# oneam/h264bsd

Hardware: AMD Instinct MI355X
Metric: 1080p macroblocks/s (higher is better)
Workload: dtype u8; 1 GPU; 256 concurrent copies of test_1920x1080.h264 per GPU (73 pictures x 8160 MB), kernel-only replay from HBM-resident frame jobs, inter+intra reconstruction + in-loop deblocking; streams_per_gpu=256, parallelism=streams/1, stream_groups=1, row_bands=library default (engine.hip TailConfig)

## Files before the change

### h264bsd_amd/csrc/engine.hip

```cpp
#include <hip/hip_runtime.h>
#include <stdio.h>
#include <stdlib.h>
#include <string.h>
#include <deque>
#include <memory>
#include <mutex>
#include <vector>
#include <algorithm>
#include "kernels.hip.h"
#include "kernels/k_tensor_out.hip.h"
#include "kernels/k_tensor_aa.hip.h"
#include "kernels/k_tensor_roi.hip.h"
#include "kernels/k_tensor_remap.hip.h"
#include "kernels/k_motion.hip.h"
#include "kernels/region_common.hip.h"
#include "kernels/k_region_stats.hip.h"
#include "kernels/k_keep.hip.h"
#include "kernels/k_blend.hip.h"
#include "kernels/k_region_change.hip.h"
#include "kernels/k_region_shift.hip.h"
#include "kernels/k_cell_maps.hip.h"
#include "kernels/k_cell_boxes.hip.h"
#include "engine.h"
#include "hip_owned.h"
// ... 293 lines not shown
    d.dbki = reinterpret_cast<const uint16_t *>(dev_blob + h->dbk_off);
    d.n_dbk = h->n_dbk;
    d.dbk = dev_dbk;
    d.cur = dev_frames + (size_t)h->cur_slot * frame_bytes;
    d.n_mbs = h->n_mbs;
    d.n_levels = h->n_intra_levels;
    d.wmb = h->width_mbs;
    d.wmb_magic = (uint32_t)(0x100000000ull / (h->width_mbs ? h->width_mbs : 1u)) + 1u;
    d.hmb = h->height_mbs;
    d.any_deblock = h->any_deblock;
    {
        const TailConfig tc = tail_config();
        const bool heavy = h->n_intra * 4u > h->n_mbs;
        d.heavy = heavy ? 1 : 0;
        d.dbk_bands = bands_for(h->height_mbs, heavy ? tc.dbk_rows_heavy : tc.dbk_rows_light);
        d.intra_bands = h->intra_down_deps ? 1 : bands_for(h->height_mbs, heavy ? tc.intra_rows_heavy : tc.intra_rows_light);
    }
    d.err = dev_err;
    d.conv_src = nullptr; d.conv_dst = nullptr; d.conv_fmt = 0; d.conv_pad = 0;
    for (uint32_t k = 0; k < FJ_MAX_SLOTS; k++) d.slot[k] = k < h->n_slots ? dev_frames + (size_t)k * frame_bytes : nullptr;
    if (shape) {
        shape->n_frames++;
        shape->max_mbs = std::max(shape->max_mbs, h->n_mbs);
        shape->max_copy = std::max(shape->max_copy, h->n_copy);
        shape->max_gen = std::max(shape->max_gen, h->n_gen);
        shape->max_gen_uni = std::max(shape->max_gen_uni, h->n_gen_uniform);
        shape->max_gen_quad = std::max(shape->max_gen_quad, h->n_gen_quad);
        shape->max_gen_rest = std::max(shape->max_gen_rest, h->n_gen - h->n_gen_uniform - h->n_gen_quad);
        shape->max_dbk = std::max(shape->max_dbk, h->n_dbk);
        shape->any_deblock |= h->any_deblock != 0;
        shape->max_levels = std::max(shape->max_levels, h->n_intra_levels);
        shape->max_w = std::max<uint32_t>(shape->max_w, h->width_mbs);
        shape->max_h = std::max<uint32_t>(shape->max_h, h->height_mbs);
        shape->any_tail |= h->n_intra_levels != 0 || h->any_deblock != 0;
        shape->n_heavy += d.heavy;
        if (h->any_deblock) (d.heavy ? shape->want_heavy : shape->want_light)[0] = std::max<uint32_t>((d.heavy ? shape->want_heavy : shape->want_light)[0], d.dbk_bands);
        if (h->n_intra_levels) (d.heavy ? shape->want_heavy : shape->want_light)[1] = std::max<uint32_t>((d.heavy ? shape->want_heavy : shape->want_light)[1], d.intra_bands);
        if (h->n_intra_levels && h->intra_down_deps) shape->intra_whole = true;
    }
}

struct TickTimers { Event ev[6]; Event sev[5]; bool on = false; bool copy_timed = false; unsigned mask = 31u; };

static void launch_kdbk(hipStream_t st, const FrameDesc *d_desc, const TickShape &s, uint32_t launches[5])
{
    hipLaunchKernelGGL(h264k::k_dbk, dim3((s.max_dbk + 64 * DBK_WG_WAVES - 1) / (64 * DBK_WG_WAVES), s.n_frames), dim3(64 * DBK_WG_WAVES), 0, st, d_desc);
    if (launches) launches[2]++;
}
template <int PATH> static void launch_inter(hipStream_t st, const FrameDesc *d_desc, uint32_t n_max, uint32_t n_frames)
{
#if INTER_LANE_BLOCKS
    if constexpr (PATH == 0) {
        if (n_max) hipLaunchKernelGGL(h264k::k_recon_inter_lb, dim3((n_max + INTER_LB_CHUNK - 1) / INTER_LB_CHUNK, n_frames), dim3(64), 0, st, d_desc);
    } else
#endif
    {
    constexpr uint32_t per_wg = INTER_WG_WAVES * h264k::inter_per_wave<PATH>();
    if (n_max) hipLaunchKernelGGL(h264k::k_recon_inter<PATH>, dim3((n_max + per_wg - 1) / per_wg, n_frames), dim3(64 * INTER_WG_WAVES), 0, st, d_desc);
    }
}
std::mutex g_tail_lds_mu;
size_t g_tail_lds[2][2][MAX_DEVICES] = {};
static int tail_prepare(hipStream_t st, int which, const BandPlan &bp, const void *fn, uint32_t **tickets)
{
    const bool banded = bp.bands > 1;
    *tickets = banded ? tickets_for(st) : nullptr;
    if (banded && !*tickets) return -1;
    int dev = 0;
    HIP_TRY(hipGetDevice(&dev));
    std::lock_guard<std::mutex> lk(g_tail_lds_mu);
    if (bp.lds > g_tail_lds[which][banded][dev]) {
        HIP_TRY(hipFuncSetAttribute(fn, hipFuncAttributeMaxDynamicSharedMemorySize, (int)bp.lds));
        g_tail_lds[which][banded][dev] = bp.lds;
    }
    return 0;
}

int launch_tick(hipStream_t st, const FrameDesc *d_desc, const TickShape &s, TickTimers *tt, uint32_t launches[5],
                unsigned stages = 7u, const SideLane *side = nullptr, unsigned long long *prof = nullptr)
{
    const bool timed = tt && tt->on;
    const unsigned tmask = timed ? tt->mask : 0u;
    auto boundary = [&](unsigned i) -> int {
        if ((((tmask << 1) | tmask) >> i) & 1u) HIP_TRY(hipEventRecord(tt->ev[i], st));
        return 0;
    };
    if (boundary(0)) return -1;
    const bool do_dbk = (stages & 4u) && s.any_deblock && s.max_dbk;
    const bool do_copy = (stages & 1u) && s.max_copy;
    const bool aside = side && side->stream && do_dbk;
    const bool copy_aside = aside && do_copy && side->copy_stream;
    if (tt) tt->copy_timed = false;
    auto launch_copy = [&](hipStream_t cs) {
        hipLaunchKernelGGL(h264k::k_copy, dim3(std::min<uint32_t>((s.max_copy + 3) / 4, COPY_WGS), s.n_frames), dim3(256), 0, cs, d_desc);
        if (launches) launches[0]++;
    };
    if (aside) {
        HIP_TRY(hipEventRecord(side->fork, st));
        HIP_TRY(hipStreamWaitEvent(side->stream, side->fork, 0));
        if (copy_aside) {
            const bool ctimed = timed && (tmask & 1u) && tt->sev[3] && tt->sev[4];
            if (tt) tt->copy_timed = ctimed;
            HIP_TRY(hipStreamWaitEvent(side->copy_stream, side->fork, 0));
            if (ctimed) HIP_TRY(hipEventRecord(tt->sev[3], side->copy_stream));
            launch_copy(side->copy_stream);
            if (ctimed) HIP_TRY(hipEventRecord(tt->sev[4], side->copy_stream));
// ... 1402 lines not shown
```

### h264bsd_amd/csrc/kernels/inter_lane_block.hip.h

```cpp
#pragma once
namespace h264k {

constexpr uint32_t lb_sel(int c) { return 0x0C000C00u | (uint32_t)c | ((uint32_t)(c + 1) << 16); }
#define LB_CP(row, c) as_s2((c) <= 6 ? perm((row)[1], (row)[0], lb_sel((c) <= 6 ? (c) : 0)) : perm((row)[2], (row)[1], lb_sel((c) <= 6 ? 0 : (c) - 4)))
#define LB_RND5(x) pk_clip(pk(0), pk(255), ((x) + pk(16)) >> pk(5))
__device__ __forceinline__ s2 lb_tap6(s2 a, s2 b, s2 c, s2 d, s2 e, s2 f) { return a + f - pk(5) * (b + e) + pk(20) * (c + d); }
__device__ __forceinline__ int lb_dot2(s2 a, s2 b, int c)
{
#if defined(__HIP_DEVICE_COMPILE__)
    return __builtin_amdgcn_sdot2(a, b, c, false);
#else
    return (int)a.x * b.x + (int)a.y * b.y + c;
#endif
}
__device__ __forceinline__ s2 lb_avg(s2 a, s2 b) { return (a + b + pk(1)) >> pk(1); }
__device__ __forceinline__ s2 lb_pick(bool c, s2 a, s2 b) { return as_s2(c ? as_u32(a) : as_u32(b)); }
__device__ __forceinline__ void lb_hsum(const uint32_t row[3], s2 &h01, s2 &h23)
{
    const s2 c0 = LB_CP(row, 0), c1 = LB_CP(row, 1), c2 = LB_CP(row, 2), c3 = LB_CP(row, 3), c4 = LB_CP(row, 4), c5 = LB_CP(row, 5), c6 = LB_CP(row, 6), c7 = LB_CP(row, 7);
    h01 = lb_tap6(c0, c1, c2, c3, c4, c5); h23 = lb_tap6(c2, c3, c4, c5, c6, c7);
}

__device__ __forceinline__ void lb_luma_whole(const uint32_t rw[9][3], s2 o[4][2])
{
// ... 108 lines not shown
}
__device__ __forceinline__ void lb_residual_pk(const uint32_t y[8], const uint32_t c[8], int qp_y, int qp_c, int dc, uint32_t r[4][4])
{
    int my, sy, mc, sc;
    lb_qp_split(qp_y, my, sy); lb_qp_split(qp_c, mc, sc);
    const s2 L0 = as_s2((uint32_t)(level_scale(my, 0) << sy) | ((uint32_t)(level_scale(mc, 0) << sc) << 16));
    const s2 L1 = as_s2((uint32_t)(level_scale(my, 1) << sy) | ((uint32_t)(level_scale(mc, 1) << sc) << 16));
    const s2 L2 = as_s2((uint32_t)(level_scale(my, 2) << sy) | ((uint32_t)(level_scale(mc, 2) << sc) << 16));
    typedef unsigned short us2 __attribute__((ext_vector_type(2)));
    auto mul = [](uint32_t a, s2 b) { us2 x, z; __builtin_memcpy(&x, &a, 4); __builtin_memcpy(&z, &b, 4); x = x * z; s2 o; __builtin_memcpy(&o, &x, 4); return o; };
    s2 f[4][4];
#pragma unroll
    for (int i = 0; i < 4; i++) {
        const s2 A = (i & 1) ? L1 : L0, B = (i & 1) ? L2 : L1;
        s2 d0 = mul(perm(c[2 * i], y[2 * i], 0x05040100u), A), d1 = mul(perm(c[2 * i], y[2 * i], 0x07060302u), B);
        const s2 d2 = mul(perm(c[2 * i + 1], y[2 * i + 1], 0x05040100u), A), d3 = mul(perm(c[2 * i + 1], y[2 * i + 1], 0x07060302u), B);
        if (i == 0) d0 = as_s2(perm((uint32_t)dc, as_u32(d0), 0x05040100u));
        const s2 e0 = d0 + d2, e1 = d0 - d2, e2 = (d1 >> pk(1)) - d3, e3 = d1 + (d3 >> pk(1));
        f[i][0] = e0 + e3; f[i][1] = e1 + e2; f[i][2] = e1 - e2; f[i][3] = e0 - e3;
    }
#pragma unroll
    for (int j = 0; j < 4; j++) {
        const s2 g0 = f[0][j] + f[2][j] + pk(32), g1 = f[0][j] - f[2][j] + pk(32);
        const s2 g2 = (f[1][j] >> pk(1)) - f[3][j], g3 = f[1][j] + (f[3][j] >> pk(1));
        r[0][j] = as_u32((g0 + g3) >> pk(6)); r[1][j] = as_u32((g1 + g2) >> pk(6)); r[2][j] = as_u32((g1 - g2) >> pk(6)); r[3][j] = as_u32((g0 - g3) >> pk(6));
    }
}
__device__ __forceinline__ bool lb_residual_32(const uint32_t lv[8], int qp, bool use_dc, int dc, int r[4][4])
{
    int m, sh;
    lb_qp_split(qp, m, sh);
    const int ls0 = level_scale(m, 0), ls1 = level_scale(m, 1), ls2 = level_scale(m, 2);
    int f[4][4];
#pragma unroll
    for (int i = 0; i < 4; i++) {
        const int lsa = (i & 1) ? ls1 : ls0, lsb = (i & 1) ? ls2 : ls1;
        int d0 = ((int)(int16_t)(lv[2 * i] & 0xFFFFu) * lsa) << sh, d1 = (((int32_t)lv[2 * i] >> 16) * lsb) << sh;
        const int d2 = ((int)(int16_t)(lv[2 * i + 1] & 0xFFFFu) * lsa) << sh, d3 = (((int32_t)lv[2 * i + 1] >> 16) * lsb) << sh;
        if (i == 0 && use_dc) d0 = dc;
        const int e0 = d0 + d2, e1 = d0 - d2, e2 = (d1 >> 1) - d3, e3 = d1 + (d3 >> 1);
        f[i][0] = e0 + e3; f[i][1] = e1 + e2; f[i][2] = e1 - e2; f[i][3] = e0 - e3;
    }
    uint32_t over = 0;
#pragma unroll
    for (int j = 0; j < 4; j++) {
        const int e0 = f[0][j] + f[2][j], e1 = f[0][j] - f[2][j], e2 = (f[1][j] >> 1) - f[3][j], e3 = f[1][j] + (f[3][j] >> 1);
        r[0][j] = (e0 + e3 + 32) >> 6; r[1][j] = (e1 + e2 + 32) >> 6; r[2][j] = (e1 - e2 + 32) >> 6; r[3][j] = (e0 - e3 + 32) >> 6;
#pragma unroll
        for (int i = 0; i < 4; i++) over |= (uint32_t)(r[i][j] + 512);
    }
    return over > 1023u;
}

}
```

### h264bsd_amd/csrc/kernels/k_recon_inter.hip.h

```cpp
#pragma once
namespace h264k {
__device__ __forceinline__ int tap6(int a, int b, int c, int d, int e, int f) { return a - 5 * (b + e) + 20 * (c + d) + f; }

__device__ __forceinline__ void luma_window_global(const uint8_t *__restrict__ p, int wmb, int w, int h, int x, int y, uint32_t rw[6][3])
{
    if (x >= 2 && x + 9 < w && y >= 2 && y + 3 < h) {
#pragma unroll
        for (int r = 0; r < 6; r++) {
            rw[r][0] = luma4_at(p, wmb, x - 2, y - 2 + r); rw[r][1] = luma4_at(p, wmb, x + 2, y - 2 + r); rw[r][2] = luma4_at(p, wmb, x + 6, y - 2 + r);
        }
    } else {
#pragma unroll
        for (int r = 0; r < 6; r++) {
            const int yy = clip3(0, h - 1, y - 2 + r);
            uint32_t a = 0, b = 0, c = 0;
#pragma unroll
            for (int i = 0; i < 4; i++) {
                a |= (uint32_t)p[luma_at(wmb, clip3(0, w - 1, x - 2 + i), yy)] << (8 * i);
                b |= (uint32_t)p[luma_at(wmb, clip3(0, w - 1, x + 2 + i), yy)] << (8 * i);
            }
            c = (uint32_t)p[luma_at(wmb, clip3(0, w - 1, x + 6), yy)];
            rw[r][0] = a; rw[r][1] = b; rw[r][2] = c;
        }
    }
// ... 437 lines not shown
#endif
    IPROF(3);
    H264K_GLOBAL uint8_t *T = cur + (size_t)mb * TILE;
    uint32_t luma_dw, chroma_dw;
    if ((ge.coded & 0x03FFFFFFu) == 0u) {
        luma_dw = perm(as_u32(pl23), as_u32(pl01), 0x06040200u);
        chroma_dw = perm(as_u32(pc23), as_u32(pc01), 0x06040200u);
    } else if (!(ge.coded & FJ_CODED_WIDE)) {
        s2 y01, y23, c01, c23;
        mb_residual_pk(ge.coded, qp_y, qp_c, lane, rrows, y01, y23, c01, c23);
        const s2 lo = pk(0), hi = pk(255);
        const s2 l01 = pk_clip(lo, hi, pl01 + y01), l23 = pk_clip(lo, hi, pl23 + y23);
        const s2 k01 = pk_clip(lo, hi, pc01 + c01), k23 = pk_clip(lo, hi, pc23 + c23);
        luma_dw = perm(as_u32(l23), as_u32(l01), 0x06040200u);
        chroma_dw = perm(as_u32(k23), as_u32(k01), 0x06040200u);
    } else {
        int ry[4], rc[4];
        report_residual_range(fd, mb_residual_compute<false>(ge.coded, qp_y, qp_c, false, coef, lane, rrows, ry, rc), lane);
        luma_dw = pack4(clip255(pl01.x + ry[0]), clip255(pl01.y + ry[1]), clip255(pl23.x + ry[2]), clip255(pl23.y + ry[3]));
        chroma_dw = pack4(clip255(pc01.x + rc[0]), clip255(pc01.y + rc[1]), clip255(pc23.x + rc[2]), clip255(pc23.y + rc[3]));
    }
#ifdef H264K_INTER_PROFILE
    asm volatile("" :: "v"(luma_dw), "v"(chroma_dw));
#endif
    IPROF(4);
    *reinterpret_cast<H264K_GLOBAL uint32_t *>(T + (by * 4 + row) * 16 + bx * 4) = luma_dw;
    if (lane < 32) {
        const int k = lane >> 2, plane = k >> 2, cbx = k & 1, cby = (k >> 1) & 1;
        *reinterpret_cast<H264K_GLOBAL uint32_t *>(T + T_CB + plane * 64 + (cby * 4 + row) * 8 + cbx * 4) = chroma_dw;
    }
    IPROF(5);
#ifdef H264K_INTER_PROFILE
    if (PATH == 0 && lane == 0 && (blockIdx.x & 63u) == 0u) {
        unsigned long long *pc64 = reinterpret_cast<unsigned long long *>(fd.err) + 8;
        for (int k = 0; k < 5; k++) atomicAdd(pc64 + k, ipt[k + 1] - ipt[k]);
        atomicAdd(pc64 + 5, 1ull);
        atomicAdd(pc64 + 6, (ge.coded & 0x03FFFFFFu) ? 1ull : 0ull);
    }
#endif
    wave_sync();
  }
}

#ifndef INTER_LANE_BLOCKS
#define INTER_LANE_BLOCKS 1
#endif
#ifndef INTER_LB_CHUNK
#define INTER_LB_CHUNK 32
#endif
#ifndef INTER_LB_OCC
#define INTER_LB_OCC 4
#endif
static_assert(INTER_LB_CHUNK % 4 == 0 && INTER_LB_CHUNK >= 4 && INTER_LB_CHUNK <= 64, "INTER_LB_CHUNK");
constexpr int LB_SLOT_LDS = 1472;
constexpr int LB_LDS = INTER_LB_CHUNK * 16 + 4 * LB_SLOT_LDS;
__global__ __launch_bounds__(64, INTER_LB_OCC) void k_recon_inter_lb(const FrameDesc *__restrict__ frames)
{
    __shared__ __attribute__((aligned(16))) uint8_t lds[LB_LDS];
    const FrameDesc &fd = FD_REF(frames, blockIdx.y);
#if INTER_XCD == 1
    const uint32_t cls8 = blockIdx.x & 7u, per8 = gridDim.x >> 3, rem8 = gridDim.x & 7u;
    const uint32_t bx_ = cls8 * per8 + (cls8 < rem8 ? cls8 : rem8) + (blockIdx.x >> 3);
#elif INTER_XCD > 1
    const uint32_t C_ = INTER_XCD, full_ = (gridDim.x / (8u * C_)) * (8u * C_);
    const uint32_t b_ = blockIdx.x, o_ = b_ % (8u * C_);
    const uint32_t bx_ = b_ >= full_ ? b_ : (b_ - o_) + (o_ & 7u) * C_ + (o_ >> 3);
#else
    const uint32_t bx_ = blockIdx.x;
#endif
    const uint32_t n_uni = fd.n_gen_uni, first = bx_ * INTER_LB_CHUNK;
    if (first >= n_uni) return;
    const uint32_t n_here = min(n_uni - first, (uint32_t)INTER_LB_CHUNK);
    const int lane = threadIdx.x & 63;
    const int wmb = fd.wmb, W = wmb * 16, H = fd.hmb * 16, CW = W >> 1, CH = H >> 1;
    const uint32_t frame_bytes = (uint32_t)wmb * fd.hmb * (uint32_t)TILE;
    const H264K_GLOBAL uint8_t *ref0 = (const H264K_GLOBAL uint8_t *)fd.slot[0];
    const H264K_GLOBAL uint8_t *cf = (const H264K_GLOBAL uint8_t *)fd.coefs;
    H264K_GLOBAL uint8_t *cur = (H264K_GLOBAL uint8_t *)fd.cur;

    {
        const bool have = (uint32_t)lane < n_here;
        uint4 e = make_uint4(0u, 0u, 0u, 0u);
        if (have) e = ld16g((const H264K_GLOBAL uint8_t *)fd.gen + 16u * (first + (uint32_t)lane));
        const int fx = (int)(e.y & 3u), fy = (int)((e.y >> 16) & 3u);
        const int cls = (fx | fy) == 0 ? 0 : fy == 0 ? 1 : fx == 0 ? 2 : (fx != 2 && fy != 2) ? 3 : 4;
        const int bin = have ? 2 * cls + ((e.w & 0x03FFFFFFu) ? 1 : 0) : 10;
        uint32_t rank = 0, seen = 0;
#pragma unroll
        for (int k = 0; k < 10; k++) {
            const unsigned long long m = __ballot(bin == k);
            const uint32_t before = __builtin_amdgcn_mbcnt_hi((uint32_t)(m >> 32), __builtin_amdgcn_mbcnt_lo((uint32_t)m, 0u));
            if (bin == k) rank = seen + before;
            seen += (uint32_t)__popcll(m);
        }
        if (have) *reinterpret_cast<uint4 *>(lds + 16u * rank) = e;
        wave_sync();
    }

#define LB_FRESH() asm volatile("" : "+v"(ln), "+v"(ge.x), "+v"(ge.y), "+v"(ge.z), "+v"(ge.w))
#define LB_LANE() const int s = ln >> 4, b = ln & 15, bx = b & 3, by = b >> 2; \
                  uint8_t *lw = lds + INTER_LB_CHUNK * 16 + s * LB_SLOT_LDS, *lc = lw + 21 * IW_STRIDE; (void)bx; (void)by; (void)lc
#pragma unroll 1
    for (uint32_t g = 0; g < n_here; g += 4) {
        int ln = lane;
        const bool on = g + (uint32_t)(lane >> 4) < n_here;
        uint4 ge = *reinterpret_cast<const uint4 *>(lds + 16u * (g + (uint32_t)(lane >> 4)));
        if (!on) ge = make_uint4(0u, 0u, 0u, 0u);
        uint32_t yl[8] = { 0u, 0u, 0u, 0u, 0u, 0u, 0u, 0u }, cl[8] = { 0u, 0u, 0u, 0u, 0u, 0u, 0u, 0u }, dcl[2] = { 0u, 0u };
        const bool any_coded = __ballot((ge.w & 0x03FFFFFFu) != 0u) != 0ull;
      {
        LB_FRESH();
        LB_LANE();
        const uint32_t mb = ge.x & 0xFFFFu, refoff = (ge.x >> 24) * frame_bytes;
        const int mvx = (int16_t)(ge.y & 0xFFFFu), mvy = (int32_t)ge.y >> 16;
        const uint32_t coded = ge.w;
        const int mby = wmb == 1 ? (int)mb : (int)__umulhi(mb, fd.wmb_magic), mbx = (int)mb - mby * wmb;
        const int xi = mbx * 16 + (mvx >> 2) - 2, yi = mby * 16 + (mvy >> 2) - 2, xs = (xi >> 4) << 4;
        const int cxi = mbx * 8 + (mvx >> 3), cyi = mby * 8 + (mvy >> 3), cxs = (cxi >> 3) << 3;
        const bool lfast = on && xi >= 0 && xi + 21 <= W && yi >= 0 && yi + 21 <= H;
        const bool cfast = on && cxi >= 0 && cxi + 9 <= CW && cyi >= 0 && cyi + 9 <= CH;

        uint4 vl[4];
// ... 27 lines not shown
            const H264K_GLOBAL uint8_t *py = ybit ? cf + yoff : ref0, *pc = cbit ? cf + coff : ref0, *pd = has_cdc ? cf + doff : ref0;
            const uint4 y0 = ld16g(py), y1 = ld16g(py + 16), c0 = ld16g(pc), c1 = ld16g(pc + 16);
            const uint2 d0 = ld8g(pd);
            const uint32_t ym = ybit ? ~0u : 0u, cm = cbit ? ~0u : 0u, dm = has_cdc ? ~0u : 0u;
            yl[0] = y0.x & ym; yl[1] = y0.y & ym; yl[2] = y0.z & ym; yl[3] = y0.w & ym; yl[4] = y1.x & ym; yl[5] = y1.y & ym; yl[6] = y1.z & ym; yl[7] = y1.w & ym;
            cl[0] = c0.x & cm; cl[1] = c0.y & cm; cl[2] = c0.z & cm; cl[3] = c0.w & cm; cl[4] = c1.x & cm; cl[5] = c1.y & cm; cl[6] = c1.z & cm; cl[7] = c1.w & cm;
            dcl[0] = d0.x & dm; dcl[1] = d0.y & dm;
        }
        if (any_edge) {
#pragma unroll
            for (int i = 0; i < 4; i++) {
                const int p = b + 16 * i, lr = (p * 43) >> 7, lk = p - 3 * lr, lx = xs + 16 * lk;
                const uint32_t first = (vl[i].x & 255u) * 0x01010101u, last = (vl[i].w >> 24) * 0x01010101u;
                if (lx < 0) vl[i] = make_uint4(first, first, first, first);
                else if (lx >= W) vl[i] = make_uint4(last, last, last, last);
            }
#pragma unroll
            for (int i = 0; i < 3; i++) {
                const int p = b + 16 * i, cp = p >= 18, rem = cp ? p - 18 : p, ck = rem & 1, cx = cxs + 8 * ck;
                const uint32_t first = (vc[i].x & 255u) * 0x01010101u, last = (vc[i].y >> 24) * 0x01010101u;
                if (cx < 0) vc[i] = make_uint2(first, first);
                else if (cx >= CW) vc[i] = make_uint2(last, last);
            }
        }
#pragma unroll
        for (int i = 0; i < 4; i++) {
            const int p = b + 16 * i, lr = (p * 43) >> 7, lk = p - 3 * lr;
            if (l_on[i]) {
                uint32_t *d32 = reinterpret_cast<uint32_t *>(lw + lr * IW_STRIDE + 16 * lk);
                d32[0] = vl[i].x; d32[1] = vl[i].y; d32[2] = vl[i].z; d32[3] = vl[i].w;
            }
        }
#pragma unroll
        for (int i = 0; i < 3; i++) {
            const int p = b + 16 * i, cp = p >= 18, rem = cp ? p - 18 : p, cr = rem >> 1, ck = rem & 1;
            if (c_on[i]) {
                uint32_t *d32 = reinterpret_cast<uint32_t *>(lc + cp * 9 * IC_STRIDE + cr * IC_STRIDE + 8 * ck);
                d32[0] = vc[i].x; d32[1] = vc[i].y;
            }
        }
        wave_sync();
      }

        s2 pl[4][2];
#pragma unroll
        for (int r = 0; r < 4; r++) pl[r][0] = pl[r][1] = pk(0);
        {
            LB_FRESH();
            LB_LANE();
            const int mvx = (int16_t)(ge.y & 0xFFFFu), mvy = (int32_t)ge.y >> 16;
            const int o = (((mvx >> 2) - 2) & 15) + 4 * bx, sh = 8 * (o & 3), fx = mvx & 3, fy = mvy & 3;
            const uint8_t *src = lw + 4 * by * IW_STRIDE + (o & ~3);
            const int cls = !on ? -1 : (fx | fy) == 0 ? 0 : fy == 0 ? 1 : fx == 0 ? 2 : (fx != 2 && fy != 2) ? 3 : 4;
            auto row = [&](uint32_t rw[3], int r, int nd) {
                const uint32_t *q = reinterpret_cast<const uint32_t *>(src + r * IW_STRIDE);
                uint32_t d[4];
#pragma unroll
                for (int k = 0; k < 4; k++) if (k <= nd) d[k] = q[k];
#pragma unroll
                for (int k = 0; k < 3; k++) rw[k] = k < nd ? (uint32_t)(((unsigned long long)d[k + 1] << 32 | d[k]) >> sh) : 0u;
            };
            if (cls == 0) {
                uint32_t rw[9][3] = {};
#pragma unroll
                for (int r = 2; r < 6; r++) row(rw[r], r, 2);
                lb_luma_whole(rw, pl);
            } else if (cls == 1) {
                uint32_t rw[9][3] = {};
#pragma unroll
                for (int r = 2; r < 6; r++) row(rw[r], r, 3);
                lb_luma_hor(rw, fx, pl);
            } else if (cls == 2) {
                uint32_t rw[9][3] = {};
#pragma unroll
                for (int r = 0; r < 9; r++) row(rw[r], r, 2);
                lb_luma_ver(rw, fy, pl);
            } else if (cls == 3) {
                uint32_t rw[9][3] = {};
#pragma unroll
                for (int r = 0; r < 9; r++) row(rw[r], r, (r >= 2 && r <= 6) ? 3 : 2);
                lb_luma_diag(rw, fx, fy, pl);
            } else if (cls == 4) {
                uint32_t rw[9][3] = {};
#pragma unroll
                for (int r = 0; r < 9; r++) row(rw[r], r, 3);
                lb_luma_centre(rw, fx, fy, pl);
            }
        }
#define LB_CHROMA_LANE() const int k8 = b & 7, plane = k8 >> 2, cbx = k8 & 1, cby = (k8 >> 1) & 1, half = b >> 3; (void)cbx
        s2 pc[2][2];
        {
            LB_FRESH();
            LB_LANE();
            LB_CHROMA_LANE();
            const int mvx = (int16_t)(ge.y & 0xFFFFu), mvy = (int32_t)ge.y >> 16;
            const int ob = ((mvx >> 3) & 7) + 4 * cbx, cfx = mvx & 7, cfy = mvy & 7;
            const uint32_t *q = reinterpret_cast<const uint32_t *>(lc + plane * 9 * IC_STRIDE + (cby * 4 + 2 * half) * IC_STRIDE + (ob & ~3));
            uint32_t lo[3], hi[3];
#pragma unroll
            for (int t = 0; t < 3; t++) {
                const uint32_t q0 = q[5 * t], q1 = q[5 * t + 1], q2 = q[5 * t + 2];
                lo[t] = __builtin_amdgcn_alignbyte(q1, q0, (uint32_t)(ob & 3)); hi[t] = __builtin_amdgcn_alignbyte(q2, q1, (uint32_t)(ob & 3));
            }
            const s2 w00 = as_s2((uint32_t)((8 - cfx) * (8 - cfy)) * 0x00010001u), w10 = as_s2((uint32_t)(cfx * (8 - cfy)) * 0x00010001u);
            const s2 w01 = as_s2((uint32_t)((8 - cfx) * cfy) * 0x00010001u), w11 = as_s2((uint32_t)(cfx * cfy) * 0x00010001u);
            lb_chroma_row(lo[0], hi[0], lo[1], hi[1], w00, w10, w01, w11, pc[0][0], pc[0][1]);
            lb_chroma_row(lo[1], hi[1], lo[2], hi[2], w00, w10, w01, w11, pc[1][0], pc[1][1]);
        }

        LB_FRESH();
        LB_LANE();
        LB_CHROMA_LANE();
        const uint32_t mb = ge.x & 0xFFFFu, coded = ge.w;
        const int qp_y = (int)FJ_GEN_QP_Y(ge.z), qp_c = (int)FJ_GEN_QP_C(ge.z);
        uint32_t ldw[4], cdw[2];
        if (!any_coded) {
#pragma unroll
            for (int r = 0; r < 4; r++) ldw[r] = perm(as_u32(pl[r][1]), as_u32(pl[r][0]), 0x06040200u);
#pragma unroll
            for (int t = 0; t < 2; t++) cdw[t] = perm(as_u32(pc[t][1]), as_u32(pc[t][0]), 0x06040200u);
        } else {
            const int dc = lb_chroma_dc(dcl[0], dcl[1], k8 & 3, qp_c);
            if (__ballot((coded & FJ_CODED_WIDE) != 0u) == 0ull) {
                uint32_t rr[4][4];
                lb_residual_pk(yl, cl, qp_y, qp_c, dc, rr);
                const s2 lo = pk(0), hi = pk(255);
#pragma unroll
                for (int r = 0; r < 4; r++) {
                    const s2 l01 = pk_clip(lo, hi, pl[r][0] + as_s2(perm(rr[r][1], rr[r][0], 0x05040100u)));
                    const s2 l23 = pk_clip(lo, hi, pl[r][1] + as_s2(perm(rr[r][3], rr[r][2], 0x05040100u)));
                    ldw[r] = perm(as_u32(l23), as_u32(l01), 0x06040200u);
                }
#pragma unroll
                for (int t = 0; t < 2; t++) {
                    const uint32_t r0 = half ? rr[2 + t][0] : rr[t][0], r1 = half ? rr[2 + t][1] : rr[t][1];
                    const uint32_t r2 = half ? rr[2 + t][2] : rr[t][2], r3 = half ? rr[2 + t][3] : rr[t][3];
                    const s2 k01 = pk_clip(lo, hi, pc[t][0] + as_s2(perm(r1, r0, 0x07060302u)));
                    const s2 k23 = pk_clip(lo, hi, pc[t][1] + as_s2(perm(r3, r2, 0x07060302u)));
                    cdw[t] = perm(as_u32(k23), as_u32(k01), 0x06040200u);
                }
            } else {
                int ry[4][4], rc[4][4];
                const bool over_y = lb_residual_32(yl, qp_y, false, 0, ry), over_c = lb_residual_32(cl, qp_c, true, dc, rc);
                report_residual_range(fd, over_y || over_c, lane);
#pragma unroll
                for (int r = 0; r < 4; r++)
                    ldw[r] = pack4(clip255(pl[r][0].x + ry[r][0]), clip255(pl[r][0].y + ry[r][1]), clip255(pl[r][1].x + ry[r][2]), clip255(pl[r][1].y + ry[r][3]));
#pragma unroll
                for (int t = 0; t < 2; t++) {
                    const int c0 = half ? rc[2 + t][0] : rc[t][0], c1 = half ? rc[2 + t][1] : rc[t][1], c2 = half ? rc[2 + t][2] : rc[t][2], c3 = half ? rc[2 + t][3] : rc[t][3];
                    cdw[t] = pack4(clip255(pc[t][0].x + c0), clip255(pc[t][0].y + c1), clip255(pc[t][1].x + c2), clip255(pc[t][1].y + c3));
                }
            }
        }
        quad_transpose4(ldw[0], ldw[1], ldw[2], ldw[3], ln);
        const uint32_t got = (uint32_t)quad_xor1((int)((b & 1) ? cdw[0] : cdw[1]));
        H264K_GLOBAL uint8_t *T = cur + (size_t)mb * TILE;
        if (on) {
            st16g(T + (4 * by + bx) * 16, make_uint4(ldw[0], ldw[1], ldw[2], ldw[3]));
            const u32x2 v = (b & 1) ? (u32x2){ got, cdw[1] } : (u32x2){ cdw[0], got };
            *(H264K_GLOBAL u32x2 *)(T + T_CB + plane * 64 + (cby * 4 + 2 * half + (b & 1)) * 8) = v;
        }
        wave_sync();
    }
#undef LB_FRESH
#undef LB_LANE
#undef LB_CHROMA_LANE
}


}
```

Measured before the change: 1.885 billion macroblocks/s.

## Add lane-quad inter reconstruction kernel for 8x8-partition path

Adds k_recon_inter_lq, a new kernel for PATH==1 (8x8-partition inter macroblocks). Each lane handles one 4x4 block, so a wave covers 16 blocks at once. Reference windows and chroma are staged cooperatively into LDS, entries are binned and ranked by class with ballots, and the residual is added using shared helpers factored out of the lane-block kernel. It replaces the generic per-wave k_recon_inter path for this partition type and aims to raise lane utilisation and reuse of loaded reference data. The cost is higher LDS use and a new indexing scheme that carries correctness risk.

```diff
diff --git a/h264bsd_amd/csrc/engine.hip b/h264bsd_amd/csrc/engine.hip
--- a/h264bsd_amd/csrc/engine.hip
+++ b/h264bsd_amd/csrc/engine.hip
@@ -369,6 +369,11 @@
 #if INTER_LANE_BLOCKS
     if constexpr (PATH == 0) {
         if (n_max) hipLaunchKernelGGL(h264k::k_recon_inter_lb, dim3((n_max + INTER_LB_CHUNK - 1) / INTER_LB_CHUNK, n_frames), dim3(64), 0, st, d_desc);
+    } else
+#endif
+#if INTER_LANE_QUADS
+    if constexpr (PATH == 1) {
+        if (n_max) hipLaunchKernelGGL(h264k::k_recon_inter_lq, dim3((n_max + INTER_LQ_CHUNK - 1) / INTER_LQ_CHUNK, n_frames), dim3(64), 0, st, d_desc);
     } else
 #endif
     {
diff --git a/h264bsd_amd/csrc/kernels/inter_lane_block.hip.h b/h264bsd_amd/csrc/kernels/inter_lane_block.hip.h
--- a/h264bsd_amd/csrc/kernels/inter_lane_block.hip.h
+++ b/h264bsd_amd/csrc/kernels/inter_lane_block.hip.h
@@ -184,4 +184,15 @@
     return over > 1023u;
 }
 
+__device__ __forceinline__ uint32_t lq_coded_mask(uint32_t q) { return (0xFu << (4u * q)) | (0x00110000u << q) | FJ_CODED_CHROMA_DC; }
+__device__ __forceinline__ int lq_window_byte(int q, int mvx) { return (8 * (q & 1) + (mvx >> 2) - 2) & 15; }
+__device__ __forceinline__ int lq_chroma_byte(int q, int mvx) { return (4 * (q & 1) + (mvx >> 3)) & 7; }
+__device__ __forceinline__ void lq_pair_rows(const uint32_t ldw[4], uint32_t got0, uint32_t got1, int jbx, uint32_t r0[2], uint32_t r1[2])
+{
+    r0[0] = jbx ? got0 : ldw[0]; r0[1] = jbx ? ldw[2] : got0;
+    r1[0] = jbx ? got1 : ldw[1]; r1[1] = jbx ? ldw[3] : got1;
 }
+__device__ __forceinline__ int lq_luma_store_offset(int q, int j) { return (8 * (q >> 1) + 4 * (j >> 1) + 2 * (j & 1)) * 16 + 8 * (q & 1); }
+__device__ __forceinline__ int lq_chroma_store_offset(int q, int j) { return T_CB + (j >> 1) * 64 + (4 * (q >> 1) + 2 * (j & 1)) * 8 + 4 * (q & 1); }
+
+}
diff --git a/h264bsd_amd/csrc/kernels/k_recon_inter.hip.h b/h264bsd_amd/csrc/kernels/k_recon_inter.hip.h
--- a/h264bsd_amd/csrc/kernels/k_recon_inter.hip.h
+++ b/h264bsd_amd/csrc/kernels/k_recon_inter.hip.h
@@ -513,22 +513,122 @@
 #define INTER_LB_OCC 4
 #endif
 static_assert(INTER_LB_CHUNK % 4 == 0 && INTER_LB_CHUNK >= 4 && INTER_LB_CHUNK <= 64, "INTER_LB_CHUNK");
+__device__ __forceinline__ uint32_t inter_chunk_of_block()
+{
+#if INTER_XCD == 1
+    const uint32_t cls8 = blockIdx.x & 7u, per8 = gridDim.x >> 3, rem8 = gridDim.x & 7u;
+    return cls8 * per8 + (cls8 < rem8 ? cls8 : rem8) + (blockIdx.x >> 3);
+#elif INTER_XCD > 1
+    const uint32_t C_ = INTER_XCD, full_ = (gridDim.x / (8u * C_)) * (8u * C_);
+    const uint32_t b_ = blockIdx.x, o_ = b_ % (8u * C_);
+    return b_ >= full_ ? b_ : (b_ - o_) + (o_ & 7u) * C_ + (o_ >> 3);
+#else
+    return blockIdx.x;
+#endif
+}
+template <int STRIDE>
+__device__ __forceinline__ void lb_luma_from_lds(const uint8_t *src, int sh, int cls, int fx, int fy, s2 pl[4][2])
+{
+    auto row = [&](uint32_t rw[3], int r, int nd) {
+        const uint32_t *q = reinterpret_cast<const uint32_t *>(src + r * STRIDE);
+        uint32_t d[4];
+#pragma unroll
+        for (int k = 0; k < 4; k++) if (k <= nd) d[k] = q[k];
+#pragma unroll
+        for (int k = 0; k < 3; k++) rw[k] = k < nd ? (uint32_t)(((unsigned long long)d[k + 1] << 32 | d[k]) >> sh) : 0u;
+    };
+    if (cls == 0) {
+        uint32_t rw[9][3] = {};
+#pragma unroll
+        for (int r = 2; r < 6; r++) row(rw[r], r, 2);
+        lb_luma_whole(rw, pl);
+    } else if (cls == 1) {
+        uint32_t rw[9][3] = {};
+#pragma unroll
+        for (int r = 2; r < 6; r++) row(rw[r], r, 3);
+        lb_luma_hor(rw, fx, pl);
+    } else if (cls == 2) {
+        uint32_t rw[9][3] = {};
+#pragma unroll
+        for (int r = 0; r < 9; r++) row(rw[r], r, 2);
+        lb_luma_ver(rw, fy, pl);
+    } else if (cls == 3) {
+        uint32_t rw[9][3] = {};
+#pragma unroll
+        for (int r = 0; r < 9; r++) row(rw[r], r, (r >= 2 && r <= 6) ? 3 : 2);
+        lb_luma_diag(rw, fx, fy, pl);
+    } else if (cls == 4) {
+        uint32_t rw[9][3] = {};
+#pragma unroll
+        for (int r = 0; r < 9; r++) row(rw[r], r, 3);
+        lb_luma_centre(rw, fx, fy, pl);
+    }
+}
+template <int DW>
+__device__ __forceinline__ void lb_chroma_from_lds(const uint32_t *q, int ob, int cfx, int cfy, s2 pc[2][2])
+{
+    uint32_t lo[3], hi[3];
+#pragma unroll
+    for (int t = 0; t < 3; t++) {
+        const uint32_t q0 = q[DW * t], q1 = q[DW * t + 1], q2 = q[DW * t + 2];
+        lo[t] = __builtin_amdgcn_alignbyte(q1, q0, (uint32_t)(ob & 3)); hi[t] = __builtin_amdgcn_alignbyte(q2, q1, (uint32_t)(ob & 3));
+    }
+    const s2 w00 = as_s2((uint32_t)((8 - cfx) * (8 - cfy)) * 0x00010001u), w10 = as_s2((uint32_t)(cfx * (8 - cfy)) * 0x00010001u);
+    const s2 w01 = as_s2((uint32_t)((8 - cfx) * cfy) * 0x00010001u), w11 = as_s2((uint32_t)(cfx * cfy) * 0x00010001u);
+    lb_chroma_row(lo[0], hi[0], lo[1], hi[1], w00, w10, w01, w11, pc[0][0], pc[0][1]);
+    lb_chroma_row(lo[1], hi[1], lo[2], hi[2], w00, w10, w01, w11, pc[1][0], pc[1][1]);
+}
+__device__ __forceinline__ void lb_add_residual(const FrameDesc &fd, int lane, bool any_coded, uint32_t coded, int qp_y, int qp_c, const uint32_t yl[8],
+                                                const uint32_t cl[8], const uint32_t dcl[2], int dci, int half, const s2 pl[4][2], const s2 pc[2][2],
+                                                uint32_t ldw[4], uint32_t cdw[2])
+{
+    if (!any_coded) {
+#pragma unroll
+        for (int r = 0; r < 4; r++) ldw[r] = perm(as_u32(pl[r][1]), as_u32(pl[r][0]), 0x06040200u);
+#pragma unroll
+        for (int t = 0; t < 2; t++) cdw[t] = perm(as_u32(pc[t][1]), as_u32(pc[t][0]), 0x06040200u);
+        return;
+    }
+    const int dc = lb_chroma_dc(dcl[0], dcl[1], dci, qp_c);
+    if (__ballot((coded & FJ_CODED_WIDE) != 0u) == 0ull) {
+        uint32_t rr[4][4];
+        lb_residual_pk(yl, cl, qp_y, qp_c, dc, rr);
+        const s2 lo = pk(0), hi = pk(255);
+#pragma unroll
+        for (int r = 0; r < 4; r++) {
+            const s2 l01 = pk_clip(lo, hi, pl[r][0] + as_s2(perm(rr[r][1], rr[r][0], 0x05040100u)));
+            const s2 l23 = pk_clip(lo, hi, pl[r][1] + as_s2(perm(rr[r][3], rr[r][2], 0x05040100u)));
+            ldw[r] = perm(as_u32(l23), as_u32(l01), 0x06040200u);
+        }
+#pragma unroll
+        for (int t = 0; t < 2; t++) {
+            const uint32_t r0 = half ? rr[2 + t][0] : rr[t][0], r1 = half ? rr[2 + t][1] : rr[t][1];
+            const uint32_t r2 = half ? rr[2 + t][2] : rr[t][2], r3 = half ? rr[2 + t][3] : rr[t][3];
+            const s2 k01 = pk_clip(lo, hi, pc[t][0] + as_s2(perm(r1, r0, 0x07060302u)));
+            const s2 k23 = pk_clip(lo, hi, pc[t][1] + as_s2(perm(r3, r2, 0x07060302u)));
+            cdw[t] = perm(as_u32(k23), as_u32(k01), 0x06040200u);
+        }
+    } else {
+        int ry[4][4], rc[4][4];
+        const bool over_y = lb_residual_32(yl, qp_y, false, 0, ry), over_c = lb_residual_32(cl, qp_c, true, dc, rc);
+        report_residual_range(fd, over_y || over_c, lane);
+#pragma unroll
+        for (int r = 0; r < 4; r++)
+            ldw[r] = pack4(clip255(pl[r][0].x + ry[r][0]), clip255(pl[r][0].y + ry[r][1]), clip255(pl[r][1].x + ry[r][2]), clip255(pl[r][1].y + ry[r][3]));
+#pragma unroll
+        for (int t = 0; t < 2; t++) {
+            const int c0 = half ? rc[2 + t][0] : rc[t][0], c1 = half ? rc[2 + t][1] : rc[t][1], c2 = half ? rc[2 + t][2] : rc[t][2], c3 = half ? rc[2 + t][3] : rc[t][3];
+            cdw[t] = pack4(clip255(pc[t][0].x + c0), clip255(pc[t][0].y + c1), clip255(pc[t][1].x + c2), clip255(pc[t][1].y + c3));
+        }
+    }
+}
 constexpr int LB_SLOT_LDS = 1472;
 constexpr int LB_LDS = INTER_LB_CHUNK * 16 + 4 * LB_SLOT_LDS;
 __global__ __launch_bounds__(64, INTER_LB_OCC) void k_recon_inter_lb(const FrameDesc *__restrict__ frames)
 {
     __shared__ __attribute__((aligned(16))) uint8_t lds[LB_LDS];
     const FrameDesc &fd = FD_REF(frames, blockIdx.y);
-#if INTER_XCD == 1
-    const uint32_t cls8 = blockIdx.x & 7u, per8 = gridDim.x >> 3, rem8 = gridDim.x & 7u;
-    const uint32_t bx_ = cls8 * per8 + (cls8 < rem8 ? cls8 : rem8) + (blockIdx.x >> 3);
-#elif INTER_XCD > 1
-    const uint32_t C_ = INTER_XCD, full_ = (gridDim.x / (8u * C_)) * (8u * C_);
-    const uint32_t b_ = blockIdx.x, o_ = b_ % (8u * C_);
-    const uint32_t bx_ = b_ >= full_ ? b_ : (b_ - o_) + (o_ & 7u) * C_ + (o_ >> 3);
-#else
-    const uint32_t bx_ = blockIdx.x;
-#endif
+    const uint32_t bx_ = inter_chunk_of_block();
     const uint32_t n_uni = fd.n_gen_uni, first = bx_ * INTER_LB_CHUNK;
     if (first >= n_uni) return;
     const uint32_t n_here = min(n_uni - first, (uint32_t)INTER_LB_CHUNK);
@@ -662,40 +762,7 @@
             const int o = (((mvx >> 2) - 2) & 15) + 4 * bx, sh = 8 * (o & 3), fx = mvx & 3, fy = mvy & 3;
             const uint8_t *src = lw + 4 * by * IW_STRIDE + (o & ~3);
             const int cls = !on ? -1 : (fx | fy) == 0 ? 0 : fy == 0 ? 1 : fx == 0 ? 2 : (fx != 2 && fy != 2) ? 3 : 4;
-            auto row = [&](uint32_t rw[3], int r, int nd) {
-                const uint32_t *q = reinterpret_cast<const uint32_t *>(src + r * IW_STRIDE);
-                uint32_t d[4];
-#pragma unroll
-                for (int k = 0; k < 4; k++) if (k <= nd) d[k] = q[k];
-#pragma unroll
-                for (int k = 0; k < 3; k++) rw[k] = k < nd ? (uint32_t)(((unsigned long long)d[k + 1] << 32 | d[k]) >> sh) : 0u;
-            };
-            if (cls == 0) {
-                uint32_t rw[9][3] = {};
-#pragma unroll
-                for (int r = 2; r < 6; r++) row(rw[r], r, 2);
-                lb_luma_whole(rw, pl);
-            } else if (cls == 1) {
-                uint32_t rw[9][3] = {};
-#pragma unroll
-                for (int r = 2; r < 6; r++) row(rw[r], r, 3);
-                lb_luma_hor(rw, fx, pl);
-            } else if (cls == 2) {
-                uint32_t rw[9][3] = {};
-#pragma unroll
-                for (int r = 0; r < 9; r++) row(rw[r], r, 2);
-                lb_luma_ver(rw, fy, pl);
-            } else if (cls == 3) {
-                uint32_t rw[9][3] = {};
-#pragma unroll
-                for (int r = 0; r < 9; r++) row(rw[r], r, (r >= 2 && r <= 6) ? 3 : 2);
-                lb_luma_diag(rw, fx, fy, pl);
-            } else if (cls == 4) {
-                uint32_t rw[9][3] = {};
-#pragma unroll
-                for (int r = 0; r < 9; r++) row(rw[r], r, 3);
-                lb_luma_centre(rw, fx, fy, pl);
-            }
+            lb_luma_from_lds<IW_STRIDE>(src, sh, cls, fx, fy, pl);
         }
 #define LB_CHROMA_LANE() const int k8 = b & 7, plane = k8 >> 2, cbx = k8 & 1, cby = (k8 >> 1) & 1, half = b >> 3; (void)cbx
         s2 pc[2][2];
@@ -706,16 +773,7 @@
             const int mvx = (int16_t)(ge.y & 0xFFFFu), mvy = (int32_t)ge.y >> 16;
             const int ob = ((mvx >> 3) & 7) + 4 * cbx, cfx = mvx & 7, cfy = mvy & 7;
             const uint32_t *q = reinterpret_cast<const uint32_t *>(lc + plane * 9 * IC_STRIDE + (cby * 4 + 2 * half) * IC_STRIDE + (ob & ~3));
-            uint32_t lo[3], hi[3];
-#pragma unroll
-            for (int t = 0; t < 3; t++) {
-                const uint32_t q0 = q[5 * t], q1 = q[5 * t + 1], q2 = q[5 * t + 2];
-                lo[t] = __builtin_amdgcn_alignbyte(q1, q0, (uint32_t)(ob & 3)); hi[t] = __builtin_amdgcn_alignbyte(q2, q1, (uint32_t)(ob & 3));
-            }
-            const s2 w00 = as_s2((uint32_t)((8 - cfx) * (8 - cfy)) * 0x00010001u), w10 = as_s2((uint32_t)(cfx * (8 - cfy)) * 0x00010001u);
-            const s2 w01 = as_s2((uint32_t)((8 - cfx) * cfy) * 0x00010001u), w11 = as_s2((uint32_t)(cfx * cfy) * 0x00010001u);
-            lb_chroma_row(lo[0], hi[0], lo[1], hi[1], w00, w10, w01, w11, pc[0][0], pc[0][1]);
-            lb_chroma_row(lo[1], hi[1], lo[2], hi[2], w00, w10, w01, w11, pc[1][0], pc[1][1]);
+            lb_chroma_from_lds<IC_STRIDE / 4>(q, ob, cfx, cfy, pc);
         }
 
         LB_FRESH();
@@ -724,45 +782,7 @@
         const uint32_t mb = ge.x & 0xFFFFu, coded = ge.w;
         const int qp_y = (int)FJ_GEN_QP_Y(ge.z), qp_c = (int)FJ_GEN_QP_C(ge.z);
         uint32_t ldw[4], cdw[2];
-        if (!any_coded) {
-#pragma unroll
-            for (int r = 0; r < 4; r++) ldw[r] = perm(as_u32(pl[r][1]), as_u32(pl[r][0]), 0x06040200u);
-#pragma unroll
-            for (int t = 0; t < 2; t++) cdw[t] = perm(as_u32(pc[t][1]), as_u32(pc[t][0]), 0x06040200u);
-        } else {
-            const int dc = lb_chroma_dc(dcl[0], dcl[1], k8 & 3, qp_c);
-            if (__ballot((coded & FJ_CODED_WIDE) != 0u) == 0ull) {
-                uint32_t rr[4][4];
-                lb_residual_pk(yl, cl, qp_y, qp_c, dc, rr);
-                const s2 lo = pk(0), hi = pk(255);
-#pragma unroll
-                for (int r = 0; r < 4; r++) {
-                    const s2 l01 = pk_clip(lo, hi, pl[r][0] + as_s2(perm(rr[r][1], rr[r][0], 0x05040100u)));
-                    const s2 l23 = pk_clip(lo, hi, pl[r][1] + as_s2(perm(rr[r][3], rr[r][2], 0x05040100u)));
-                    ldw[r] = perm(as_u32(l23), as_u32(l01), 0x06040200u);
-                }
-#pragma unroll
-                for (int t = 0; t < 2; t++) {
-                    const uint32_t r0 = half ? rr[2 + t][0] : rr[t][0], r1 = half ? rr[2 + t][1] : rr[t][1];
-                    const uint32_t r2 = half ? rr[2 + t][2] : rr[t][2], r3 = half ? rr[2 + t][3] : rr[t][3];
-                    const s2 k01 = pk_clip(lo, hi, pc[t][0] + as_s2(perm(r1, r0, 0x07060302u)));
-                    const s2 k23 = pk_clip(lo, hi, pc[t][1] + as_s2(perm(r3, r2, 0x07060302u)));
-                    cdw[t] = perm(as_u32(k23), as_u32(k01), 0x06040200u);
-                }
-            } else {
-                int ry[4][4], rc[4][4];
-                const bool over_y = lb_residual_32(yl, qp_y, false, 0, ry), over_c = lb_residual_32(cl, qp_c, true, dc, rc);
-                report_residual_range(fd, over_y || over_c, lane);
-#pragma unroll
-                for (int r = 0; r < 4; r++)
-                    ldw[r] = pack4(clip255(pl[r][0].x + ry[r][0]), clip255(pl[r][0].y + ry[r][1]), clip255(pl[r][1].x + ry[r][2]), clip255(pl[r][1].y + ry[r][3]));
-#pragma unroll
-                for (int t = 0; t < 2; t++) {
-                    const int c0 = half ? rc[2 + t][0] : rc[t][0], c1 = half ? rc[2 + t][1] : rc[t][1], c2 = half ? rc[2 + t][2] : rc[t][2], c3 = half ? rc[2 + t][3] : rc[t][3];
-                    cdw[t] = pack4(clip255(pc[t][0].x + c0), clip255(pc[t][0].y + c1), clip255(pc[t][1].x + c2), clip255(pc[t][1].y + c3));
-                }
-            }
-        }
+        lb_add_residual(fd, lane, any_coded, coded, qp_y, qp_c, yl, cl, dcl, k8 & 3, half, pl, pc, ldw, cdw);
         quad_transpose4(ldw[0], ldw[1], ldw[2], ldw[3], ln);
         const uint32_t got = (uint32_t)quad_xor1((int)((b & 1) ? cdw[0] : cdw[1]));
         H264K_GLOBAL uint8_t *T = cur + (size_t)mb * TILE;
@@ -778,5 +798,223 @@
 #undef LB_CHROMA_LANE
 }
 
-
-}
+#ifndef INTER_LANE_QUADS
+#define INTER_LANE_QUADS 1
+#endif
+#ifndef INTER_LQ_CHUNK
+#define INTER_LQ_CHUNK 8
+#endif
+#ifndef INTER_LQ_OCC
+#define INTER_LQ_OCC 4
+#endif
+#ifndef INTER_LQ_WSTRIDE
+#define INTER_LQ_WSTRIDE 32
+#endif
+#ifndef INTER_LQ_CSTRIDE
+#define INTER_LQ_CSTRIDE 16
+#endif
+static_assert(INTER_LQ_CHUNK % 4 == 0 && INTER_LQ_CHUNK >= 4 && INTER_LQ_CHUNK <= 64, "INTER_LQ_CHUNK");
+constexpr int LQ_ROUNDS = (INTER_LQ_CHUNK + 15) / 16;
+constexpr int LQ_W_STRIDE = INTER_LQ_WSTRIDE, LQ_C_STRIDE = INTER_LQ_CSTRIDE;
+static_assert(LQ_W_STRIDE >= 32 && LQ_W_STRIDE % 4 == 0 && LQ_C_STRIDE >= 16 && LQ_C_STRIDE % 4 == 0, "staged rows");
+constexpr int LQ_SLOT_LDS = 13 * LQ_W_STRIDE + 2 * 5 * LQ_C_STRIDE;
+constexpr int LQ_ITEMS_LDS = INTER_LQ_CHUNK * 4 * 16;
+constexpr int LQ_LDS = LQ_ITEMS_LDS + 16 * LQ_SLOT_LDS;
+static_assert(INTER_LQ_CHUNK * 32 + LQ_ROUNDS * 64 <= 16 * LQ_SLOT_LDS, "the fetched entries lie where the windows will");
+__global__ __launch_bounds__(64, INTER_LQ_OCC) void k_recon_inter_lq(const FrameDesc *__restrict__ frames)
+{
+    __shared__ __attribute__((aligned(16))) uint8_t lds[LQ_LDS];
+    const FrameDesc &fd = FD_REF(frames, blockIdx.y);
+    const uint32_t n_quad = fd.n_gen_quad, first = inter_chunk_of_block() * INTER_LQ_CHUNK;
+    if (first >= n_quad) return;
+    const uint32_t n_here = min(n_quad - first, (uint32_t)INTER_LQ_CHUNK), n_items = 4u * n_here;
+    const int lane = threadIdx.x & 63;
+    const int wmb = fd.wmb, W = wmb * 16, H = fd.hmb * 16, CW = W >> 1, CH = H >> 1;
+    const uint32_t frame_bytes = (uint32_t)wmb * fd.hmb * (uint32_t)TILE;
+    const H264K_GLOBAL uint8_t *ref0 = (const H264K_GLOBAL uint8_t *)fd.slot[0];
+    const H264K_GLOBAL uint8_t *cf = (const H264K_GLOBAL uint8_t *)fd.coefs;
+    H264K_GLOBAL uint8_t *cur = (H264K_GLOBAL uint8_t *)fd.cur;
+
+    {
+        uint4 *raw_e = reinterpret_cast<uint4 *>(lds + LQ_ITEMS_LDS), *raw_mv = raw_e + INTER_LQ_CHUNK;
+        uint32_t *raw_ref = reinterpret_cast<uint32_t *>(raw_mv + INTER_LQ_CHUNK);
+        if ((uint32_t)lane < n_here) {
+            const uint4 e = ld16g((const H264K_GLOBAL uint8_t *)fd.gen + 16u * (fd.n_gen_uni + first + (uint32_t)lane));
+            const H264K_GLOBAL uint32_t *mvc = (const H264K_GLOBAL uint32_t *)fd.mvx + 16 * (size_t)e.y;
+            const uint32_t refs = *(const H264K_GLOBAL uint32_t *)((const H264K_GLOBAL uint8_t *)fd.recs + sizeof(FjMbRec) * (size_t)(e.x & 0xFFFFu) + offsetof(FjMbRec, ref_slot));
+            raw_e[lane] = e;
+            raw_mv[lane] = make_uint4(mvc[0], mvc[2], mvc[8], mvc[10]);
+            raw_ref[lane] = refs;
+        }
+        wave_sync();
+        uint4 it[LQ_ROUNDS];
+        int bin[LQ_ROUNDS];
+        bool have[LQ_ROUNDS];
+#pragma unroll
+        for (int r = 0; r < LQ_ROUNDS; r++) {
+            const uint32_t ent = 16u * r + ((uint32_t)lane >> 2), q = (uint32_t)lane & 3u;
+            have[r] = ent < n_here;
+            const uint4 e = raw_e[ent], m4 = raw_mv[ent];
+            const uint32_t mv = q == 0u ? m4.x : q == 1u ? m4.y : q == 2u ? m4.z : m4.w;
+            it[r] = make_uint4((e.x & 0xFFFFu) | (q << 16) | (((raw_ref[ent] >> (8u * q)) & 255u) << 24), mv, e.z, e.w);
+            const int fx = (int)(mv & 3u), fy = (int)((mv >> 16) & 3u);
+            const int cls = (fx | fy) == 0 ? 0 : fy == 0 ? 1 : fx == 0 ? 2 : (fx != 2 && fy != 2) ? 3 : 4;
+            bin[r] = have[r] ? 2 * cls + ((e.w & lq_coded_mask(q)) ? 1 : 0) : 10;
+        }
+        uint32_t rank[LQ_ROUNDS] = {}, seen = 0;
+#pragma unroll
+        for (int k = 0; k < 10; k++)
+#pragma unroll
+            for (int r = 0; r < LQ_ROUNDS; r++) {
+                const unsigned long long m = __ballot(bin[r] == k);
+                const uint32_t before = __builtin_amdgcn_mbcnt_hi((uint32_t)(m >> 32), __builtin_amdgcn_mbcnt_lo((uint32_t)m, 0u));
+                if (bin[r] == k) rank[r] = seen + before;
+                seen += (uint32_t)__popcll(m);
+            }
+        wave_sync();
+#pragma unroll
+        for (int r = 0; r < LQ_ROUNDS; r++)
+            if (have[r]) *reinterpret_cast<uint4 *>(lds + 16u * rank[r]) = it[r];
+        wave_sync();
+    }
+
+#define LQ_FRESH() asm volatile("" : "+v"(ln), "+v"(ge.x), "+v"(ge.y), "+v"(ge.z), "+v"(ge.w))
+#define LQ_LANE() const int s = ln >> 2, j = ln & 3, jbx = j & 1, jby = j >> 1, qd = (int)((ge.x >> 16) & 3u), plane = j >> 1, half = j & 1; \
+                  uint8_t *lw = lds + LQ_ITEMS_LDS + s * LQ_SLOT_LDS, *lc = lw + 13 * LQ_W_STRIDE; (void)jbx; (void)jby; (void)qd; (void)plane; (void)half; (void)lc
+#pragma unroll 1
+    for (uint32_t g = 0; g < n_items; g += 16) {
+        int ln = lane;
+        const bool on = g + (uint32_t)(lane >> 2) < n_items;
+        uint4 ge = *reinterpret_cast<const uint4 *>(lds + 16u * (g + (uint32_t)(lane >> 2)));
+        if (!on) ge = make_uint4(0u, 0u, 0u, 0u);
+        uint32_t yl[8] = { 0u, 0u, 0u, 0u, 0u, 0u, 0u, 0u }, cl[8] = { 0u, 0u, 0u, 0u, 0u, 0u, 0u, 0u }, dcl[2] = { 0u, 0u };
+        const bool any_coded = __ballot((ge.w & lq_coded_mask((ge.x >> 16) & 3u)) != 0u) != 0ull;
+      {
+        LQ_FRESH();
+        LQ_LANE();
+        const uint32_t mb = ge.x & 0xFFFFu, refoff = (ge.x >> 24) * frame_bytes;
+        const int mvx = (int16_t)(ge.y & 0xFFFFu), mvy = (int32_t)ge.y >> 16;
+        const uint32_t coded = ge.w;
+        const int mby = wmb == 1 ? (int)mb : (int)__umulhi(mb, fd.wmb_magic), mbx = (int)mb - mby * wmb;
+        const int xi = mbx * 16 + 8 * (qd & 1) + (mvx >> 2) - 2, yi = mby * 16 + 8 * (qd >> 1) + (mvy >> 2) - 2, xs = (xi >> 4) << 4;
+        const int cxi = mbx * 8 + 4 * (qd & 1) + (mvx >> 3), cyi = mby * 8 + 4 * (qd >> 1) + (mvy >> 3), cxs = (cxi >> 3) << 3;
+        const bool lfast = on && xi >= 0 && xi + 13 <= W && yi >= 0 && yi + 13 <= H;
+        const bool cfast = on && cxi >= 0 && cxi + 5 <= CW && cyi >= 0 && cyi + 5 <= CH;
+
+        uint4 vl[7];
+        uint2 vc[5];
+        bool l_on[7], c_on[5];
+        const bool any_edge = __ballot(on && !(lfast && cfast)) != 0ull;
+#pragma unroll
+        for (int i = 0; i < 7; i++) {
+            const int p = j + 4 * i, lr = p >> 1, lk = p & 1;
+            const int lx = clip3(0, W - 16, xs + 16 * lk), yy = clip3(0, H - 1, yi + lr);
+            l_on[i] = on && p < 26 && (lk == 0 || xi - xs >= 4);
+            const uint32_t off = refoff + (uint32_t)((yy >> 4) * wmb + (lx >> 4)) * (uint32_t)TILE + (uint32_t)((yy & 15) << 4);
+            vl[i] = ld16g(ref0 + (l_on[i] ? off : 0u));
+        }
+#pragma unroll
+        for (int i = 0; i < 5; i++) {
+            const int p = j + 4 * i, cp = p >= 10, rem = cp ? p - 10 : p, cr = rem >> 1, ck = rem & 1;
+            const int cx = clip3(0, CW - 8, cxs + 8 * ck), yy = clip3(0, CH - 1, cyi + cr);
+            c_on[i] = on;
+            const uint32_t off = refoff + (uint32_t)((yy >> 3) * wmb + (cx >> 3)) * (uint32_t)TILE + (uint32_t)(T_CB + (cp << 6) + ((yy & 7) << 3));
+            vc[i] = ld8g(ref0 + (c_on[i] ? off : 0u));
+        }
+        if (any_coded) {
+            const int z = 4 * qd + j, k8 = 4 * plane + qd;
+            const uint32_t cidx = FJ_GEN_COEF_IDX(ge.z), nl = (uint32_t)__popc(coded & 0xFFFFu), has_cdc = (coded >> 25) & 1u;
+            const bool ybit = (coded >> z) & 1u, cbit = (coded >> (16 + k8)) & 1u;
+            const uint32_t yoff = 32u * (cidx + (uint32_t)__popc(coded & ((1u << z) - 1u)));
+            const uint32_t coff = 32u * (cidx + nl + has_cdc + (uint32_t)__popc((coded >> 16) & ((1u << k8) - 1u)));
+            const uint32_t doff = 32u * (cidx + nl) + 8u * (uint32_t)plane;
+            const H264K_GLOBAL uint8_t *py = ybit ? cf + yoff : ref0, *pc = cbit ? cf + coff : ref0, *pd = has_cdc ? cf + doff : ref0;
+            const uint4 y0 = ld16g(py), y1 = ld16g(py + 16), c0 = ld16g(pc), c1 = ld16g(pc + 16);
+            const uint2 d0 = ld8g(pd);
+            const uint32_t ym = ybit ? ~0u : 0u, cm = cbit ? ~0u : 0u, dm = has_cdc ? ~0u : 0u;
+            yl[0] = y0.x & ym; yl[1] = y0.y & ym; yl[2] = y0.z & ym; yl[3] = y0.w & ym; yl[4] = y1.x & ym; yl[5] = y1.y & ym; yl[6] = y1.z & ym; yl[7] = y1.w & ym;
+            cl[0] = c0.x & cm; cl[1] = c0.y & cm; cl[2] = c0.z & cm; cl[3] = c0.w & cm; cl[4] = c1.x & cm; cl[5] = c1.y & cm; cl[6] = c1.z & cm; cl[7] = c1.w & cm;
+            dcl[0] = d0.x & dm; dcl[1] = d0.y & dm;
+        }
+        if (any_edge) {
+#pragma unroll
+            for (int i = 0; i < 7; i++) {
+                const int p = j + 4 * i, lk = p & 1, lx = xs + 16 * lk;
+                const uint32_t first = (vl[i].x & 255u) * 0x01010101u, last = (vl[i].w >> 24) * 0x01010101u;
+                if (lx < 0) vl[i] = make_uint4(first, first, first, first);
+                else if (lx >= W) vl[i] = make_uint4(last, last, last, last);
+            }
+#pragma unroll
+            for (int i = 0; i < 5; i++) {
+                const int p = j + 4 * i, ck = p & 1, cx = cxs + 8 * ck;
+                const uint32_t first = (vc[i].x & 255u) * 0x01010101u, last = (vc[i].y >> 24) * 0x01010101u;
+                if (cx < 0) vc[i] = make_uint2(first, first);
+                else if (cx >= CW) vc[i] = make_uint2(last, last);
+            }
+        }
+#pragma unroll
+        for (int i = 0; i < 7; i++) {
+            const int p = j + 4 * i, lr = p >> 1, lk = p & 1;
+            if (l_on[i]) {
+                uint32_t *d32 = reinterpret_cast<uint32_t *>(lw + lr * LQ_W_STRIDE + 16 * lk);
+                d32[0] = vl[i].x; d32[1] = vl[i].y; d32[2] = vl[i].z; d32[3] = vl[i].w;
+            }
+        }
+#pragma unroll
+        for (int i = 0; i < 5; i++) {
+            const int p = j + 4 * i, cp = p >= 10, rem = cp ? p - 10 : p, cr = rem >> 1, ck = rem & 1;
+            if (c_on[i]) {
+                uint32_t *d32 = reinterpret_cast<uint32_t *>(lc + cp * 5 * LQ_C_STRIDE + cr * LQ_C_STRIDE + 8 * ck);
+                d32[0] = vc[i].x; d32[1] = vc[i].y;
+            }
+        }
+        wave_sync();
+      }
+
+        s2 pl[4][2];
+#pragma unroll
+        for (int r = 0; r < 4; r++) pl[r][0] = pl[r][1] = pk(0);
+        {
+            LQ_FRESH();
+            LQ_LANE();
+            const int mvx = (int16_t)(ge.y & 0xFFFFu), mvy = (int32_t)ge.y >> 16;
+            const int o = lq_window_byte(qd, mvx) + 4 * jbx, sh = 8 * (o & 3), fx = mvx & 3, fy = mvy & 3;
+            const uint8_t *src = lw + 4 * jby * LQ_W_STRIDE + (o & ~3);
+            const int cls = !on ? -1 : (fx | fy) == 0 ? 0 : fy == 0 ? 1 : fx == 0 ? 2 : (fx != 2 && fy != 2) ? 3 : 4;
+            lb_luma_from_lds<LQ_W_STRIDE>(src, sh, cls, fx, fy, pl);
+        }
+        s2 pc[2][2];
+        {
+            LQ_FRESH();
+            LQ_LANE();
+            const int mvx = (int16_t)(ge.y & 0xFFFFu), mvy = (int32_t)ge.y >> 16;
+            const int ob = lq_chroma_byte(qd, mvx), cfx = mvx & 7, cfy = mvy & 7;
+            const uint32_t *q = reinterpret_cast<const uint32_t *>(lc + plane * 5 * LQ_C_STRIDE + 2 * half * LQ_C_STRIDE + (ob & ~3));
+            lb_chroma_from_lds<LQ_C_STRIDE / 4>(q, ob, cfx, cfy, pc);
+        }
+
+        LQ_FRESH();
+        LQ_LANE();
+        const uint32_t mb = ge.x & 0xFFFFu, coded = ge.w;
+        const int qp_y = (int)FJ_GEN_QP_Y(ge.z), qp_c = (int)FJ_GEN_QP_C(ge.z);
+        uint32_t ldw[4], cdw[2];
+        lb_add_residual(fd, lane, any_coded, coded, qp_y, qp_c, yl, cl, dcl, qd, half, pl, pc, ldw, cdw);
+        uint32_t r0[2], r1[2];
+        lq_pair_rows(ldw, (uint32_t)quad_xor1((int)(jbx ? ldw[0] : ldw[2])), (uint32_t)quad_xor1((int)(jbx ? ldw[1] : ldw[3])), jbx, r0, r1);
+        H264K_GLOBAL uint8_t *T = cur + (size_t)mb * TILE;
+        if (on) {
+            H264K_GLOBAL uint8_t *L = T + lq_luma_store_offset(qd, j);
+            *(H264K_GLOBAL u32x2 *)L = (u32x2){ r0[0], r0[1] };
+            *(H264K_GLOBAL u32x2 *)(L + 16) = (u32x2){ r1[0], r1[1] };
+            H264K_GLOBAL uint8_t *C = T + lq_chroma_store_offset(qd, j);
+            *(H264K_GLOBAL uint32_t *)C = cdw[0];
+            *(H264K_GLOBAL uint32_t *)(C + 8) = cdw[1];
+        }
+        wave_sync();
+    }
+#undef LQ_FRESH
+#undef LQ_LANE
+}
+
+
+}
```

Measured after the change: 1.980 billion macroblocks/s, median of 6. 1.05x the previous value.
